# MuMuJun97/semantic_slam_mapping

Hardware: AMD Instinct MI355X
Metric: frames/sec semantic-mapping, 640x480 RGB-D (higher is better)
Workload: dtype u8; 1 GPU; configs[1]: synthetic 640x480 RGB-D + precomputed 12-class masks, 1k frames per GPU, ORB 1000 kp/frame, 5 ref frames, leaf 0.10 m; frames_per_gpu=1000, frames_all_gpus=1000, batch_frames=250, matcher_halo_frames=0, parallelism=single GPU

## Files before the change

### semantic_slam_mapping_amd/csrc/kernels_map.hip

```cpp
#include "ssm_internal.h"
#include <cstring>
#include <cmath>

#define MK_W 64
#define MK_H 16
__global__ void __launch_bounds__(256)
mask_kernel(const uint8_t* __restrict__ sem, int w, int h, int tiles_x, uint8_t* __restrict__ mask)
{
    __shared__ uint8_t m0[MK_H + 4][MK_W + 4];
    __shared__ uint8_t m1[MK_H + 4][MK_W];
    const int tx0 = (blockIdx.x % tiles_x) * MK_W, ty0 = (blockIdx.x / tiles_x) * MK_H;
    const uint8_t* s = sem + (size_t)blockIdx.y * w * h * 3;
    for (int i = threadIdx.x; i < (MK_H + 4) * (MK_W + 4); i += 256) {
        const int ly = i / (MK_W + 4), lx = i - ly * (MK_W + 4);
        const int gx = tx0 + lx - 2, gy = ty0 + ly - 2;
        uint8_t v = 0;
        if (gx >= 0 && gx < w && gy >= 0 && gy < h) {
            const uint8_t* p = s + ((size_t)gy * w + gx) * 3;
            const int b = p[0], g = p[1], r = p[2];
            v = ((b == 0 && g == 64 && r == 64) || (b == 192 && g == 128 && r == 0)) ? 255 : 0;
        }
        m0[ly][lx] = v;
    }
    __syncthreads();
// ... 311 lines not shown
    vox_insert_kernel<<<(int)blocks, 256, 0, s>>>(pts, n_dev, n_max, 1.0f / leaf, tab, cap_log2, counters);
    return hipGetLastError();
}
template <int CTRL, int ROW_MASK>
__device__ __forceinline__ int dpp_mov0(int v) { return __builtin_amdgcn_update_dpp(0, v, CTRL, ROW_MASK, 0xF, false); }
template <int CTRL, int ROW_MASK>
__device__ __forceinline__ long long dpp_mov0_ll(long long v)
{
    const int lo = dpp_mov0<CTRL, ROW_MASK>((int)(unsigned)(unsigned long long)v), hi = dpp_mov0<CTRL, ROW_MASK>((int)((unsigned long long)v >> 32));
    return (long long)(((unsigned long long)(unsigned)hi << 32) | (unsigned)lo);
}
struct RunAcc { long long sx, sy, sz; uint32_t r, g, b, n; };
__device__ __forceinline__ void run_scan(RunAcc& a, int lane, int start)
{
#define RS_STEP(CTRL, MASK, COND)                                                                                   \
    {   const long long tx = dpp_mov0_ll<CTRL, MASK>(a.sx), ty = dpp_mov0_ll<CTRL, MASK>(a.sy), tz = dpp_mov0_ll<CTRL, MASK>(a.sz); \
        const uint32_t t1 = (uint32_t)dpp_mov0<CTRL, MASK>((int)a.r), t2 = (uint32_t)dpp_mov0<CTRL, MASK>((int)a.g);             \
        const uint32_t t3 = (uint32_t)dpp_mov0<CTRL, MASK>((int)a.b), t4 = (uint32_t)dpp_mov0<CTRL, MASK>((int)a.n);             \
        if (COND) { a.sx += tx; a.sy += ty; a.sz += tz; a.r += t1; a.g += t2; a.b += t3; a.n += t4; } }
    const int li = lane & 15, row = lane >> 4;
    RS_STEP(0x111, 0xF, (li >= 1 && lane - 1 >= start))
    RS_STEP(0x112, 0xF, (li >= 2 && lane - 2 >= start))
    RS_STEP(0x114, 0xF, (li >= 4 && lane - 4 >= start))
    RS_STEP(0x118, 0xF, (li >= 8 && lane - 8 >= start))
    RS_STEP(0x142, 0xA, ((row & 1) && start < 16 * row))
    RS_STEP(0x143, 0xC, (row >= 2 && start < 32))
#undef RS_STEP
}
__device__ __forceinline__ long long f64_to_ll_rn(double v)
{
    const double M = 6755399441055744.0;
    return __double_as_longlong(v + M) - __double_as_longlong(M);
}
__device__ __forceinline__ uint32_t label_hash_entry(int k)
{
    switch (k) {
        case 10: return (0u << 24) | 128u | (128u << 8) | (128u << 16);   case 1:  return (1u << 24) | 0u | (0u << 8) | (128u << 16);
        case 2:  return (2u << 24) | 128u | (192u << 8) | (192u << 16);   case 9:  return (3u << 24) | 0u | (69u << 8) | (255u << 16);
        case 4:  return (4u << 24) | 128u | (64u << 8) | (128u << 16);    case 13: return (5u << 24) | 222u | (40u << 8) | (60u << 16);
        case 14: return (6u << 24) | 0u | (128u << 8) | (128u << 16);     case 11: return (7u << 24) | 128u | (128u << 8) | (192u << 16);
        case 3:  return (8u << 24) | 128u | (64u << 8) | (64u << 16);     case 12: return (9u << 24) | 128u | (0u << 8) | (64u << 16);
        case 7:  return (10u << 24) | 0u | (64u << 8) | (64u << 16);      case 15: return (11u << 24) | 192u | (128u << 8) | (0u << 16);
    }
    return 0xFF000001u;
}
#define MS_SLOTS 256
#ifndef MS_MINB
#define MS_MINB 4
#endif
#define MS_CH 3
struct LdsVox { long long key, sx, sy, sz; unsigned r, g, b, n; unsigned hist[6]; };
__device__ __forceinline__ uint32_t label_of_bgr24(uint32_t bgr)
{
    switch (bgr) {
        case 128u | (128u << 8) | (128u << 16): return 0;   case 0u | (0u << 8) | (128u << 16): return 1;
        case 128u | (192u << 8) | (192u << 16): return 2;   case 0u | (69u << 8) | (255u << 16): return 3;
        case 128u | (64u << 8) | (128u << 16): return 4;    case 222u | (40u << 8) | (60u << 16): return 5;
        case 0u | (128u << 8) | (128u << 16): return 6;     case 128u | (128u << 8) | (192u << 16): return 7;
        case 128u | (64u << 8) | (64u << 16): return 8;     case 128u | (0u << 8) | (64u << 16): return 9;
        case 0u | (64u << 8) | (64u << 16): return 10;      case 192u | (128u << 8) | (0u << 16): return 11;
    }
    return 255;
}
__device__ __forceinline__ void vox_direct(long long key, uint32_t lab, long long sx, long long sy, long long sz, unsigned r, unsigned g, unsigned b, unsigned n,
                ssm_voxel* tab, int cap_log2, int32_t* counters, uint32_t* occ)
{
// ... 98 lines not shown
            const int i = j < own0 ? j : j + (own1 - own0);
            const int rr = (int)__umulhi((uint32_t)i, mul_wpr), gy = ry0 + rr;
            uint32_t bits = 0;
            if (gy >= 0 && gy < h) {
                const uint4* p = reinterpret_cast<const uint4*>(sem + ((size_t)by * words + (size_t)((long long)ry0 * wpr + i)) * 48);
                const uint4 a = p[0], b = p[1], c = p[2];
                const uint32_t d[13] = {a.x, a.y, a.z, a.w, b.x, b.y, b.z, b.w, c.x, c.y, c.z, c.w, 0u};
#pragma unroll
                for (int k = 0; k < 16; k++) {
                    const int o = 3 * k;
                    const uint32_t bgr = ((o & 3) ? __builtin_amdgcn_alignbyte(d[(o >> 2) + 1], d[o >> 2], o & 3) : d[o >> 2]) & 0xFFFFFFu;
                    bits |= (uint32_t)(bgr == (0u | (64u << 8) | (64u << 16)) || bgr == (192u | (128u << 8) | (0u << 16))) << k;
                }
            }
            cbits[i] = (uint16_t)bits;
        }
    }
    for (int i = tid; i < MS_SLOTS; i += 256) {
        lt[i].key = SSM_VOX_EMPTY; lt[i].sx = 0; lt[i].sy = 0; lt[i].sz = 0; lt[i].r = lt[i].g = lt[i].b = lt[i].n = 0;
#pragma unroll
        for (int k = 0; k < 6; k++) lt[i].hist[k] = 0;
    }
    if (tid == 0) s_npts = 0;
    __syncthreads();
    if (!REDO && s_skip) return;
    uint32_t* occ = reinterpret_cast<uint32_t*>(tab + (1u << cap_log2));
    int kept = 0; bool out_of_range = false;
    double T[12];
    const bool hasT = pose != nullptr;
    if (hasT) { const double* P = pose + (size_t)by * 16;
#pragma unroll
        for (int j = 0; j < 4; j++) { T[3*j] = P[4*j]; T[3*j+1] = P[4*j+1]; T[3*j+2] = P[4*j+2]; } }
    const int dmax = maxd >= 65535.0 ? 65535 : (int)maxd;
#pragma unroll 1
    for (int ch = 0; ch < MS_CH; ch++) {
    const int wbase = (bx * MS_CH + ch) * 256 + wv * 64;
    const int wi = wbase + lane;
    uint32_t keepbits = 0;
    uint32_t lab4[2] = {labs[0][0], labs[0][1]};
#pragma unroll
    for (int c_ = 1; c_ < MS_CH; c_++) { lab4[0] = ch == c_ ? labs[c_][0] : lab4[0]; lab4[1] = ch == c_ ? labs[c_][1] : lab4[1]; }
    if (wi < words) {
        const size_t gw = (size_t)by * words + wi;
        const int gy = (int)__umulhi((uint32_t)wi, mul_wpr), xw = wi - gy * wpr;
        const uint4* pd = reinterpret_cast<const uint4*>(depth + gw * 16);
        const uint4 D0 = pd[0], D1 = pd[1];
        const uint16_t* cb = cbits + (gy - ry0 - 2) * wpr + xw;
        uint32_t vl = 0, vc = 0, vr = 0;
#pragma unroll
        for (int r5 = 0; r5 < 5; r5++) { vc |= cb[r5 * wpr]; if (xw > 0) vl |= cb[r5 * wpr - 1]; if (xw + 1 < wpr) vr |= cb[r5 * wpr + 1]; }
        const unsigned long long win = (unsigned long long)vl | ((unsigned long long)vc << 16) | ((unsigned long long)vr << 32);
        const uint32_t moving = (uint32_t)((win >> 14) | (win >> 15) | (win >> 16) | (win >> 17) | (win >> 18)) & 0xFFFFu;
        const uint32_t dd[8] = {D0.x, D0.y, D0.z, D0.w, D1.x, D1.y, D1.z, D1.w};
#pragma unroll
        for (int k = 0; k < 16; k++) {
            const int d = (dd[k >> 1] >> (16 * (k & 1))) & 0xFFFF;
            const uint32_t lab = (lab4[k >> 3] >> (4 * (k & 7))) & 15u;
            const bool gated = (0x805u >> lab) & 1u;
            keepbits |= (uint32_t)(d != 0 && d <= dmax && !gated) << k;
        }
        keepbits &= ~moving;
    }
    const uint32_t cnt = __popc(keepbits);
    uint32_t incl = cnt;
    incl += (uint32_t)__builtin_amdgcn_update_dpp(0, (int)incl, 0x111, 0xF, 0xF, false);
    incl += (uint32_t)__builtin_amdgcn_update_dpp(0, (int)incl, 0x112, 0xF, 0xF, false);
    incl += (uint32_t)__builtin_amdgcn_update_dpp(0, (int)incl, 0x114, 0xF, 0xF, false);
    incl += (uint32_t)__builtin_amdgcn_update_dpp(0, (int)incl, 0x118, 0xF, 0xF, false);
    incl += (uint32_t)__builtin_amdgcn_update_dpp(0, (int)incl, 0x142, 0xA, 0xF, false);
    incl += (uint32_t)__builtin_amdgcn_update_dpp(0, (int)incl, 0x143, 0xC, 0xF, false);
    const int V = __builtin_amdgcn_readlane((int)incl, 63);
    kept += (int)cnt;
    {
        int base = (int)(incl - cnt);
#pragma unroll
        for (int k = 0; k < 16; k++)
            if ((keepbits >> k) & 1u) vlist[wv][base++] = (uint16_t)((lane << 4) | k | (((lab4[k >> 3] >> (4 * (k & 7))) & 15u) << 10));
    }
    const int P = (V + 63) >> 6;
    long long k0 = -2, k1 = -2; uint32_t l0 = 255, l1 = 255; RunAcc a0, a1;
    a0.sx = a0.sy = a0.sz = 0; a0.r = a0.g = a0.b = a0.n = 0; a1 = a0;
    __builtin_amdgcn_wave_barrier();
    struct PixIn { uint32_t ent; int d; uint32_t c01, c2; };
    auto fetch = [&](int e, PixIn& q) {
        q.ent = vlist[wv][min(e, V - 1)];
        const int sl = (q.ent >> 4) & 63, k = q.ent & 15;
        const size_t gp = ((size_t)by * words + wbase + sl) * 16 + k;
        q.d = depth[gp];
        uint16_t c01; __builtin_memcpy(&c01, rgb + gp * 3, 2);
        q.c01 = c01; q.c2 = rgb[gp * 3 + 2];
    };
    auto pixel = [&](int e, const PixIn& q, long long& key, uint32_t& lab, RunAcc& p) {
        const uint32_t ent = q.ent;
        const int sl = (ent >> 4) & 63, k = ent & 15;
        lab = (ent >> 10) == 15u ? 255u : (ent >> 10);
        const int d = q.d;
        const uint32_t cbgr = q.c01 | (q.c2 << 16);
        const int wip = wbase + sl;
        const int gy = (int)__umulhi((uint32_t)wip, mul_wpr), gx = ((wip - gy * wpr) << 4) + k;
        const double yf = (double)gy - cam.cy;
        float x, y, z;
        if (FASTDIV) {
            z = (float)markstein_div((double)d, cam.scale, md.rscale);
            x = (float)markstein_div(((double)gx - cam.cx) * (double)z, cam.fx, md.rfx);
            y = (float)markstein_div(yf * (double)z, cam.fy, md.rfy);
        } else {
            z = (float)((double)d / cam.scale);
            x = (float)(((double)gx - cam.cx) * (double)z / cam.fx);
            y = (float)(yf * (double)z / cam.fy);
        }
        float ox = x, oy = y, oz = z;
        if (hasT) {
            const double X = x, Y = y, Z = z;
            ox = (float)(T[0] * X + T[3] * Y + T[6] * Z + T[9]);
            oy = (float)(T[1] * X + T[4] * Y + T[7] * Z + T[10]);
            oz = (float)(T[2] * X + T[5] * Y + T[8] * Z + T[11]);
        }
        const float fi = floorf(ox * inv_leaf), fj = floorf(oy * inv_leaf), fk = floorf(oz * inv_leaf);
        const long long vi = (long long)(int)fi + (1 << 20), vj = (long long)(int)fj + (1 << 20), vk = (long long)(int)fk + (1 << 20);
        key = (vk << 42) | (vj << 21) | vi;
        if (!(fabsf(fi) < 1048576.0f && fabsf(fj) < 1048576.0f && fabsf(fk) < 1048576.0f)) { key = -1; if (e < V) out_of_range = true; }
        p.sx = f64_to_ll_rn((double)ox * 16777216.0); p.sy = f64_to_ll_rn((double)oy * 16777216.0); p.sz = f64_to_ll_rn((double)oz * 16777216.0);
        p.b = cbgr & 255; p.g = (cbgr >> 8) & 255; p.r = cbgr >> 16; p.n = 1;
    };
    auto accumulate = [&](long long key, uint32_t lab, const RunAcc& p) {
        if (k1 == -2 && (k0 == -2 || (k0 == key && l0 == lab))) {
            k0 = key; l0 = lab; a0.sx += p.sx; a0.sy += p.sy; a0.sz += p.sz; a0.r += p.r; a0.g += p.g; a0.b += p.b; a0.n += 1;
        } else if (k1 == -2 || (k1 == key && l1 == lab)) {
            k1 = key; l1 = lab; a1.sx += p.sx; a1.sy += p.sy; a1.sz += p.sz; a1.r += p.r; a1.g += p.g; a1.b += p.b; a1.n += 1;
        } else {
            if (k1 >= 0) lds_vox_update(lt, k1, l1, a1, tab, cap_log2, counters, occ);
            k1 = key; l1 = lab; a1 = p;
        }
    };
    constexpr int MS2_UN = 2;
    PixIn cur[MS2_UN], nxt[MS2_UN];
    if (P > 0) {
#pragma unroll
        for (int u = 0; u < MS2_UN; u++) fetch(lane * P + u, nxt[u]);
    }
#pragma unroll 1
    for (int i = 0; i < P; i += MS2_UN) {
        long long kk[MS2_UN]; uint32_t ll[MS2_UN]; RunAcc pp[MS2_UN];
#pragma unroll
        for (int u = 0; u < MS2_UN; u++) { cur[u] = nxt[u]; fetch(lane * P + i + MS2_UN + u, nxt[u]); }
#pragma unroll
        for (int u = 0; u < MS2_UN; u++) pixel(lane * P + i + u, cur[u], kk[u], ll[u], pp[u]);
#pragma unroll
        for (int u = 0; u < MS2_UN; u++) if (i + u < P && lane * P + i + u < V) accumulate(kk[u], ll[u], pp[u]);
    }
    if (k0 >= 0) lds_vox_update(lt, k0, l0, a0, tab, cap_log2, counters, occ);
    if (k1 >= 0) lds_vox_update(lt, k1, l1, a1, tab, cap_log2, counters, occ);
    __builtin_amdgcn_wave_barrier();
    }
#pragma unroll
    for (int o = 32; o > 0; o >>= 1) kept += __shfl_xor(kept, o, 64);
    if (lane == 0 && kept) atomicAdd(&s_npts, kept);
    if (__ballot(out_of_range) && lane == 0) atomicOr(&counters[1], 2);
    __syncthreads();
    for (int i = tid; i < MS_SLOTS; i += 256) {
        if (lt[i].key == SSM_VOX_EMPTY) continue;
        ssm_voxel* v = vox_find_or_insert(tab, cap_log2, lt[i].key, counters, occ);
        if (__builtin_expect(!v, 0)) { vox_overflow_packed(counters, lt[i].key, lt[i].sx, lt[i].sy, lt[i].sz, lt[i].r, lt[i].g, lt[i].b, lt[i].n, lt[i].hist); continue; }
        vox_add(v, lt[i].sx, lt[i].sy, lt[i].sz, lt[i].r, lt[i].g, lt[i].b, lt[i].n);
#pragma unroll
        for (int c = 0; c < 12; c++) { const uint32_t k = (lt[i].hist[c >> 1] >> (16 * (c & 1))) & 0xFFFF; if (k) atomicAdd(&v->hist[c], k); }
    }
    if (tid == 0 && s_npts) atomicAdd(&npoints[by], s_npts);
}
bool k_map_div(const ssm_camera& cam, MapDiv& md)
{
    md.rscale = 1.0 / cam.scale; md.rfx = 1.0 / cam.fx; md.rfy = 1.0 / cam.fy;
    auto plain = [](double f) {
        uint64_t b; memcpy(&b, &f, 8);
        const uint64_t man = b & 0xFFFFFFFFFFFFFull; const int ex = (int)((b >> 52) & 0x7FF);
        return f > 0 && ex > 0 && ex < 0x7FF && man != 0xFFFFFFFFFFFFFull;
    };
    bool ok = plain(cam.scale) && plain(cam.fx) && plain(cam.fy);
    for (int d = 0; d < 65536 && ok; d++) {
        double q = (double)d * md.rscale; q = std::fma(std::fma(-q, cam.scale, (double)d), md.rscale, q); q = std::fma(std::fma(-q, cam.scale, (double)d), md.rscale, q);
        if (q != (double)d / cam.scale) ok = false;
    }
    return ok;
}
int k_map_fuse_blocks_per_frame(int w, int h) { const int words = (w >> 4) * h; return (words + 256 * MS_CH - 1) / (256 * MS_CH); }
int k_map_fuse_block_records(void) { return MS_CH * 4096; }
int k_map_fuse_resident_blocks(void) { return 256 * MS2_MINB; }
int k_map_fuse_skip_cap(void) { return MS2_SKIP_CAP; }
hipError_t k_map_fuse(const uint16_t* depth, const uint8_t* rgb, const uint8_t* sem, const double* pose, int n, int w, int h,
                      ssm_camera cam, const MapDiv& md, bool fast, double max_distance, float leaf,
                      ssm_voxel* tab, int cap_log2, int32_t* counters, int32_t* npoints, hipStream_t s, int32_t* skip, int hw, int tag, const int32_t* redo_ids, int nredo)
{
    const int wpr = w >> 4, words = wpr * h;
    if (!((long long)words * wpr < (1ll << 32) && wpr <= 256)) return hipErrorInvalidValue;
    if (nredo <= 0) { const hipError_t e = hipMemsetAsync(npoints, 0, sizeof(int32_t) * n, s); if (e != hipSuccess) return e; }
    const int gx = (words + 256 * MS_CH - 1) / (256 * MS_CH);
    const dim3 grid(gx, n);
    const uint32_t mul_wpr = (uint32_t)(((1ull << 32) + wpr - 1) / wpr);
    const double maxd = max_distance * cam.scale; const float il = 1.0f / leaf;
    if (nredo > 0) {
        int32_t* ids = const_cast<int32_t*>(redo_ids);
        if (fast) map_stream2_kernel<true, true><<<nredo, 256, 0, s>>>(depth, rgb, sem, pose, w, h, cam, md, maxd, il, tab, cap_log2, counters, npoints, mul_wpr, ids, 0, tag, gx);
        else map_stream2_kernel<false, true><<<nredo, 256, 0, s>>>(depth, rgb, sem, pose, w, h, cam, md, maxd, il, tab, cap_log2, counters, npoints, mul_wpr, ids, 0, tag, gx);
    } else {
        if (fast) map_stream2_kernel<true, false><<<grid, 256, 0, s>>>(depth, rgb, sem, pose, w, h, cam, md, maxd, il, tab, cap_log2, counters, npoints, mul_wpr, skip, hw, tag, gx);
        else map_stream2_kernel<false, false><<<grid, 256, 0, s>>>(depth, rgb, sem, pose, w, h, cam, md, maxd, il, tab, cap_log2, counters, npoints, mul_wpr, skip, hw, tag, gx);
    }
    return hipGetLastError();
}

__global__ void vox_merge_kernel(const ssm_voxel* __restrict__ src, int n, ssm_voxel* __restrict__ tab, int cap_log2, int32_t* __restrict__ counters)
{
    uint32_t* occ = reinterpret_cast<uint32_t*>(tab + (1u << cap_log2));
    const int i = blockIdx.x * blockDim.x + threadIdx.x;
    if (i >= n) return;
    const ssm_voxel sv = src[i];
    ssm_voxel* v = vox_find_or_insert(tab, cap_log2, sv.key, counters, occ);
    if (!v) { if (g_voxel* o = vox_overflow_slot(counters)) vox_store_record(o, sv); return; }
    vox_add(v, sv.sx, sv.sy, sv.sz, sv.sr, sv.sg, sv.sb, sv.n);
    for (int c = 0; c < 12; c++) if (sv.hist[c]) atomicAdd(&v->hist[c], sv.hist[c]);
// ... 135 lines not shown
```

### semantic_slam_mapping_amd/csrc/ssm_abi.hip

```cpp
#include "ssm_ctx.h"
#include <set>

static const int8_t k_default_pattern[1024] = {
#include "orb_pattern.inc"
};
thread_local std::string g_create_err;

static int fast_scored_cells(int a, int b, int n, int origin, int cell)
{
    const int s0 = a - 1 > SSM_EDGE ? a - 1 : SSM_EDGE, s1 = (b + 1 < n - SSM_EDGE ? b + 1 : n - SSM_EDGE) - 1;
    return (s1 - origin - 3) / cell - (s0 - origin - 3) / cell + 1;
}
static int build_geometry(const ssm_config& c, OrbGeom& g, std::string& err)
{
    memset(&g, 0, sizeof(g));
    if (c.orb_levels < 1 || c.orb_levels > SSM_MAX_LEVELS) { err = "orb_levels must be 1..12"; return SSM_E_INVAL; }
    if (c.orb_features < 1) { err = "orb_features must be >= 1"; return SSM_E_INVAL; }
    if (c.orb_iniThFAST < 1 || c.orb_minThFAST < 1 || c.orb_minThFAST > 254 || c.orb_iniThFAST > 254) { err = "FAST thresholds must be 1..254"; return SSM_E_INVAL; }
    if (c.width < 64 || c.height < 64 || c.width > 4000 || c.height > 4000) { err = "frame size must be 64..4000"; return SSM_E_INVAL; }
    if (!(c.orb_scale > 1.0f)) { err = "orb_scale must be > 1"; return SSM_E_INVAL; }
    g.nlevels = c.orb_levels; g.W = c.width; g.H = c.height; g.ini_th = c.orb_iniThFAST; g.min_th = c.orb_minThFAST;
    const double scaleFactor = (double)c.orb_scale;
    float sf[SSM_MAX_LEVELS], inv[SSM_MAX_LEVELS];
    sf[0] = 1.0f;
// ... 136 lines not shown
}

extern "C" void ssm_config_default(ssm_config* c)
{
    memset(c, 0, sizeof(*c));
    c->width = 640; c->height = 480;
    c->orb_features = 2000; c->orb_scale = 1.2f; c->orb_levels = 8; c->orb_iniThFAST = 20; c->orb_minThFAST = 7;
    c->knn_match_ratio = 0.8; c->tracker_ref_frames = 5;
    c->mapper_resolution = 0.1; c->mapper_max_distance = 40;
    c->camera.cx = 318.6; c->camera.cy = 255.3; c->camera.fx = 517.3; c->camera.fy = 516.5; c->camera.scale = 1000.0;
    c->max_batch = 16; c->voxel_capacity_log2 = 20; c->brief_pattern = nullptr;
    c->voxel_max_capacity_log2 = 28; c->sgbm_form = 0; c->sgbm_streams = 0; c->stereo_batch = 0;
}
extern "C" const char* ssm_version(void) { return "ssm_hip 0.1 (gfx950)"; }
extern "C" const char* ssm_last_error(const ssm_ctx* c) { return c ? c->err.c_str() : g_create_err.c_str(); }

static int orb_work_alloc(ssm_ctx* c, OrbWork& w)
{
    const OrbGeom& g = c->g; const int B = c->B;
    DALLOC(c, w.pyr, (size_t)B * g.pyr_bytes + 16); DALLOC(c, w.blur, (size_t)B * g.blur_bytes);
    DALLOC(c, w.ncand, k_fast_ncand_pad(B, g) + k_fast_cellmax_ints(B, g)); w.cellmax = w.ncand + k_fast_ncand_pad(B, g);
    DALLOC(c, w.cand, (size_t)B * g.cand_total); DALLOC(c, w.nodeof, (size_t)B * g.cand_total);
    DALLOC(c, w.sel, (size_t)B * g.sel_total); DALLOC(c, w.nsel, (size_t)B * g.nlevels);
    DALLOC(c, w.kpaux, (size_t)B * g.sel_total * 2);
    return SSM_OK;
}
static int ctx_init(ssm_ctx* c)
{
    const ssm_config& cfg = c->cfg; const OrbGeom& g = c->g; const int B = c->B, W = g.W, H = g.H;
    HIPCHK(c, c->main.stream.ensure());
    c->dev.id = c->device;
    { int v = 0; if (hipDeviceGetAttribute(&v, hipDeviceAttributeMultiprocessorCount, c->device) == hipSuccess && v > 0) c->dev.cus = v; }
    { int v = 0; if (hipDeviceGetAttribute(&v, hipDeviceAttributeMaxSharedMemoryPerBlock, c->device) == hipSuccess && v > 0) c->dev.max_lds = v; }
    c->map_div_exact = k_map_div(cfg.camera, c->map_div);
    DALLOC(c, c->d_pattern, 1024);
    HIPCHK(c, hipMemcpy(c->d_pattern, cfg.brief_pattern ? cfg.brief_pattern : k_default_pattern, 1024, hipMemcpyHostToDevice));
    {   float pf[1024]; const int8_t* src = cfg.brief_pattern ? cfg.brief_pattern : k_default_pattern;
        for (int i = 0; i < 1024; i++) pf[i] = (float)src[i];
        { const char* e = getenv("SSM_BLUR_VARIANT"); c->blur_mfma = !(e && atoi(e) == 0); }
        { std::vector<uint8_t> bt(blur_mfma_table_bytes(c->g)); blur_mfma_tables(c->g, bt.data());
          DALLOC(c, c->d_blur_tab, bt.size());
          HIPCHK(c, hipMemcpy(c->d_blur_tab, bt.data(), bt.size(), hipMemcpyHostToDevice)); }
        DALLOC(c, c->d_pattern_f, 1024);
        HIPCHK(c, hipMemcpy(c->d_pattern_f, pf, sizeof(pf), hipMemcpyHostToDevice)); }
    std::vector<int32_t> yall[SSM_MAX_LEVELS]; bool streaming[SSM_MAX_LEVELS] = {}, wide_ok[SSM_MAX_LEVELS] = {};
    for (int l = 1; l < g.nlevels; l++) {
        std::vector<int32_t> xo, yo; std::vector<int16_t> xa, ya;
        resize_tables(g.L[l-1].w, g.L[l].w, xo, xa); resize_tables(g.L[l-1].h, g.L[l].h, yo, ya);
        yall[l] = yo;
        std::vector<uint32_t> xg, xg8; bool fits = false, fits8 = false;
        pyramid_xgroups(xo, xa, ya, g.L[l].w, g.L[l].stride, g.L[l-1].stride, xg, xg8, fits, fits8);
        while (yo.size() & 3) { yo.push_back(yo.back()); ya.push_back(ya[ya.size() - 2]); ya.push_back(ya[ya.size() - 2]); }
        DALLOC(c, c->d_xofs[l], xo.size()); DALLOC(c, c->d_xa[l], xa.size()); DALLOC(c, c->d_yofs[l], yo.size()); DALLOC(c, c->d_ya[l], ya.size());
        HIPCHK(c, hipMemcpy(c->d_xofs[l], xo.data(), xo.size() * 4, hipMemcpyHostToDevice));
        HIPCHK(c, hipMemcpy(c->d_xa[l], xa.data(), xa.size() * 2, hipMemcpyHostToDevice));
        HIPCHK(c, hipMemcpy(c->d_yofs[l], yo.data(), yo.size() * 4, hipMemcpyHostToDevice));
        HIPCHK(c, hipMemcpy(c->d_ya[l], ya.data(), ya.size() * 2, hipMemcpyHostToDevice));
        if (fits) {
            DALLOC(c, c->d_xgrp[l], xg.size());
            HIPCHK(c, hipMemcpy(c->d_xgrp[l], xg.data(), xg.size() * 4, hipMemcpyHostToDevice));
            streaming[l] = true;
        }
        if (fits && fits8) {
            DALLOC(c, c->d_xgrp8[l], xg8.size());
            HIPCHK(c, hipMemcpy(c->d_xgrp8[l], xg8.data(), xg8.size() * 4, hipMemcpyHostToDevice));
            wide_ok[l] = true;
// ... 813 lines not shown
```

### semantic_slam_mapping_amd/csrc/ssm_internal.h

```cpp
#pragma once
#include <hip/hip_runtime.h>
#include <stdint.h>
#include <vector>
#include "../../include/ssm_hip.h"

#define SSM_MAX_LEVELS 12
#define SSM_EDGE 19
#define SSM_HALF_PATCH 15
#define SSM_PATCH 31
#define SSM_MAX_NODES 1024
#define SSM_VOX_EMPTY ((int64_t)-1)

struct LevelGeom {
    int w, h, stride;
    int img_off;
    int nCols, nRows, wCell, hCell;
    int cell_off;
    int tile_off, tiles_x;
    int ftile_off, ftiles_x;
    int ftw, fth;
    int nfeat;
    int cand_off, cand_cap;
    int sel_off, sel_cap;
    int minBX, minBY, maxBX, maxBY;
// ... 4 lines not shown
    int boff;
    int bt_off, bt_x, bt_units_off;
    uint32_t mulW, mulH;
};
__host__ __device__ inline int blur_off(int boff, int stride, int x, int y) { return boff + (((y >> 3) * (stride >> 4) + (x >> 4)) << 7) + ((y & 7) << 4) + (x & 15); }
#define FT_W 126
#define FT_H 32
#define FT_SW (FT_W + 2)
#define FT_SH (FT_H + 2)
#define FT_PW 144
#define FT_PH (FT_SH + 6)
#define FT_SST 132
#define FT_BW 32
#define FT_STAGE ((FT_PH * FT_PW) / 8)
#define FT_LDS_BYTES (4 * 8 + FT_PH * FT_PW + (FT_SH + 2) * FT_SST + 2 * FT_SW * FT_SH + 2 * (FT_SW + 2) + 2 * (FT_SH + 2) + 4 * 64 + 4 * 4 + 4 * 3)
__host__ __device__ inline void ftile_rect(const LevelGeom& L, int tx, int ty, int& x0, int& x1, int& y0, int& y1)
{
    x0 = SSM_EDGE + tx * L.ftw; x1 = x0 + L.ftw < L.w - SSM_EDGE ? x0 + L.ftw : L.w - SSM_EDGE;
    y0 = SSM_EDGE + ty * L.fth; y1 = y0 + L.fth < L.h - SSM_EDGE ? y0 + L.fth : L.h - SSM_EDGE;
}
struct OrbGeom {
    int nlevels, W, H;
    int pyr_bytes;
    int cells_total, cand_total, sel_total, tiles_total, ftiles_total;
    int blur_bytes;
    int bt_total, bt_units_total;
    int cap;
    int ini_th, min_th;
    int umax[SSM_HALF_PATCH + 1];
    LevelGeom L[SSM_MAX_LEVELS];
};
typedef uint2 cand_t;

struct DeviceInfo { int id = 0, cus = 256, max_lds = 160 * 1024; };
hipError_t allow_dynamic_lds(const void* fn, size_t bytes, int limit);

hipError_t k_gray(const uint8_t* img, int channels, int n, const OrbGeom& g, uint8_t* pyr, hipStream_t s);
hipError_t k_copy_gray_strided(const uint8_t* img, int stride, const OrbGeom& g, uint8_t* pyr, hipStream_t s);
hipError_t k_pyramid(int n, const OrbGeom& g, uint8_t* pyr, const int32_t* const* xofs, const int16_t* const* xa,
                     const int32_t* const* yofs, const int16_t* const* ya, const void* const* xgroups, hipStream_t s);
#define PB_MAX_LDS (80 * 1024)
struct PyrBandArgs {
    const void* xg[SSM_MAX_LEVELS]; const int32_t* yofs[SSM_MAX_LEVELS]; const int16_t* ya[SSM_MAX_LEVELS]; uint32_t mulq0, mulg[SSM_MAX_LEVELS]; int buf1;
    uint32_t wide;
};
__host__ __device__ inline int pyr_wide(const PyrBandArgs& t, int l) { return (int)(t.wide >> l) & 1; }
struct PyrBandPlan { int bands = 0; size_t lds = 0; void* d_tab = nullptr; PyrBandArgs args = {}; };
struct PyrItems { int groups, c0, nblk, items; };
__host__ __device__ inline PyrItems pyr_items(int stride, int wide, int comp_lo, int comp_hi)
{
    PyrItems it; it.groups = stride >> (wide ? 3 : 2); it.c0 = comp_lo & ~3; it.nblk = ((comp_hi - it.c0) >> 2) + 1;
    it.items = it.groups * it.nblk;
    return it;
}
__host__ __device__ inline int pyr_item_run(int i, uint32_t mulg) { return (int)(((uint64_t)(uint32_t)i * mulg) >> 32); }
#define PYR_SLACK 16
void pyramid_xgroups(const std::vector<int32_t>& xo, const std::vector<int16_t>& xa, const std::vector<int16_t>& ya, int dw, int dstride, int sstride,
                     std::vector<uint32_t>& xg4, std::vector<uint32_t>& xg8, bool& fits4, bool& fits8);
bool pyramid_band_choose(const OrbGeom& g, const std::vector<int32_t>* yofs, const bool* streaming, const bool* wide_ok, bool batch, std::vector<int32_t>& tab, PyrBandPlan& p);
bool pyramid_band_plan(const OrbGeom& g, const std::vector<int32_t>* yofs, const bool* streaming, const bool* wide_ok, int bands, std::vector<int32_t>& tab, PyrBandPlan& p);
hipError_t k_pyramid_bands(const uint8_t* img, int channels, int n, const OrbGeom& g, uint8_t* pyr, const PyrBandPlan& p,
                           const int32_t* const* yofs, const int16_t* const* ya, const void* const* xgroups, const void* const* xgroups8, hipStream_t s);
int pyramid_block_threads();
hipError_t k_blur(int n, const OrbGeom& g, const uint8_t* pyr, uint8_t* blur, hipStream_t s);
#define BLUR_ROWS 58
hipError_t k_blur_mfma(int n, const OrbGeom& g, const uint8_t* pyr, uint8_t* blur, const void* tab, hipStream_t s);
size_t blur_mfma_table_bytes(const OrbGeom& g);
// ... 5 lines not shown
                    uint32_t* sel, int32_t* nsel, int32_t* status, hipStream_t s);
hipError_t k_describe(int n, const OrbGeom& g, const uint8_t* pyr, const uint8_t* blur, const uint32_t* sel,
                      const int32_t* nsel, const float* pattern_f , const uint16_t* depth, ssm_camera cam, void* kpaux ,
                      ssm_keypoint* kps, uint8_t* desc, float* pos3d, int32_t* nkp, hipStream_t s);

struct MatchPair { int32_t qoff, nq, toff, nt, out_slot; };
hipError_t k_match_pairs(const uint8_t* desc, const MatchPair* pairs, int npairs, double ratio, int cap,
                         ssm_dmatch* out, int32_t* nout, int32_t* knn_idx, int32_t* knn_dist, hipStream_t s);
hipError_t k_match_seq(const uint8_t* desc, const int32_t* nkp, int f0, int n, int R, int hist, double ratio, int cap,
                       ssm_dmatch* out, int32_t* nout, int32_t* pend , hipStream_t s);

#define SSM_MATCH_DESC_BYTES 128
hipError_t k_match_expand(const uint8_t* desc, const int32_t* nkp, int row0, int nrows, int cap, int capT, uint8_t* eq, uint8_t* et, hipStream_t s);
hipError_t k_match_seq_mfma(const uint8_t* eq, const uint8_t* et, const int32_t* nkp, int f0, int n, int R, int hist, double ratio, int cap, int capT,
                            void* knn , ssm_dmatch* out, int32_t* nout, hipStream_t s);

hipError_t k_moving_mask(const uint8_t* sem, int n, int w, int h, uint8_t* mask, hipStream_t s);
hipError_t k_backproject(const uint16_t* depth, const uint8_t* rgb, const uint8_t* sem, const uint8_t* mask,
                         const double* pose, int n, int w, int h, ssm_camera cam, double max_distance,
                         int32_t* chunk_cnt, int64_t* chunk_off, int32_t* npoints, int64_t* total,
                         ssm_point* out, hipStream_t s);
int backproject_chunks(int w, int h);

hipError_t k_voxel_clear(ssm_voxel* tab, int cap_log2, int32_t* counters, hipStream_t s);
hipError_t k_voxel_insert(const ssm_point* pts, const int64_t* n_dev, int64_t n_max, float leaf, ssm_voxel* tab,
                          int cap_log2, int32_t* counters, hipStream_t s);
struct MapDiv { double rscale, rfx, rfy; };
bool k_map_div(const ssm_camera& cam, MapDiv& md);
hipError_t k_map_fuse(const uint16_t* depth, const uint8_t* rgb, const uint8_t* sem, const double* pose, int n, int w, int h,
                      ssm_camera cam, const MapDiv& md, bool exact, double max_distance, float leaf,
                      ssm_voxel* tab, int cap_log2, int32_t* counters, int32_t* npoints, hipStream_t s, int32_t* skip, int hw, int tag, const int32_t* redo_ids, int nredo);
int k_map_fuse_blocks_per_frame(int w, int h);
int k_map_fuse_block_records(void);
int k_map_fuse_resident_blocks(void);
int k_map_fuse_skip_cap(void);
hipError_t k_voxel_merge(const ssm_voxel* src, int n, ssm_voxel* tab, int cap_log2, int32_t* counters, hipStream_t s);
hipError_t k_voxel_rehash(const ssm_voxel* src, int src_cap_log2, ssm_voxel* tab, int cap_log2, int32_t* counters, hipStream_t s);
hipError_t k_voxel_compact(const ssm_voxel* tab, int cap_log2, ssm_voxel* out, int32_t* n_out, hipStream_t s);
hipError_t k_voxel_gather_points(const ssm_voxel* compact, const uint32_t* order, int n, ssm_point* out, hipStream_t s);
hipError_t k_voxel_gather_table(const ssm_voxel* compact, const uint32_t* order, int n, ssm_voxel* out, hipStream_t s);
hipError_t k_voxel_bounds(const ssm_point* pts, int n, float* minmax6, hipStream_t s);
hipError_t k_cloud_transform(const ssm_point* src, int n, const double* T, ssm_point* dst, hipStream_t s);
hipError_t voxel_sort_pairs(void* tmp, size_t* tmp_bytes, const ssm_voxel* compact, int n, uint64_t* keys_a, uint64_t* keys_b,
                            uint32_t* idx_a, uint32_t* idx_b, hipStream_t s);

hipError_t k_synth(uint64_t seed, int first, int n, int w, int h, uint8_t* bgr, uint16_t* depth, uint8_t* sem,
                   uint8_t* lab, double* pose, hipStream_t s);

hipError_t k_segnet_prep(const uint8_t* bgr, int n, int sw, int sh, int dw, int dh, const int32_t* xofs, const int16_t* xa,
                         const int32_t* yofs, const int16_t* ya, void* out_f16, hipStream_t s);
#define CONV_QUEUE_INTS 1024
hipError_t k_segnet_begin(int* tiles, hipStream_t s);
hipError_t k_segnet_conv(const void* in, const void* wt, const float* scale, const float* shift, void* out, int n, int H, int W,
                         int CinPad, int Cout, int relu, const DeviceInfo& dev, int* tiles, hipStream_t s, const void* wt_wino = nullptr);
size_t k_sgbm_workspace_bytes(int w, int h, const ssm_sgbm_params& p, int nb, int form_cfg);
bool sgbm_cost_geometry(int D, int SW, int* TX_out, size_t* lds_out);
struct SgFan;
hipError_t k_sgbm(const uint8_t* left, const uint8_t* right, int w, int h, int nb, const ssm_sgbm_params& p, void* workspace, size_t ws_bytes, int16_t* disp_out, int raw_only,
                  const DeviceInfo& dev, SgFan& fan, hipStream_t s, int* fail_flag = nullptr, int form_cfg = 0, int concurrent = 1);
hipError_t k_sgbm_post(const int16_t* src, int16_t* dst, int w, int h, int nb, int op, int newVal, int maxSpeckleSize, int maxDiff, int* parent, int* count, hipStream_t s);
hipError_t k_sgbm_depth(const int16_t* disp, int w, int h, int nb, double baseline, double cu, double cv, double f, double roix, double roiy, double roiz, double scale,
                        int* min_scratch , uint16_t* depth, hipStream_t s);
hipError_t k_vo_estimate(const ssm_pmatch* m, int n, const ssm_vo_params& P, const int32_t* samples, int iters,
                         double* tr_all, int32_t* count, double* tr_out, int32_t* inliers, int32_t* result, hipStream_t s);
hipError_t k_vo_estimate_batch(const ssm_pmatch* m_all, int stride, const int32_t* n_all, int nb, const ssm_vo_params& P, const uint32_t* rand_stream, int iters,
                               int32_t* consumed, int32_t* rand_off, double* tr_all, int32_t* count, double* tr_out, int32_t* inliers, int32_t* result, hipStream_t s);
hipError_t k_segnet_conv_argmax(const void* in, const void* wt, const float* scale, const float* shift, uint8_t* labels, int n, int H, int W,
// ... 37 lines not shown
```

### semantic_slam_mapping_amd/csrc/ssm_map.hip

```cpp
#include "ssm_ctx.h"
#include <algorithm>

int table_alloc(ssm_ctx* c, hipStream_t s, VoxTable& t, int cap_log2, const VoxTable* lists)
{
    if (!lists) lists = &t;
    t.cap_log2 = cap_log2;
    { const int r = t.tab.alloc_bytes(c, t.bytes()); if (r) return r; }
    const size_t slots = (size_t)1 << cap_log2;
    t.occ = reinterpret_cast<uint32_t*>(t.tab + slots); t.counters = reinterpret_cast<int32_t*>(t.occ + slots);
    HIPCHK(c, k_voxel_clear(t.tab, -cap_log2, t.counters, s));
    struct { int32_t cap, pad; ssm_voxel* buf; } tail = { lists->ovf ? lists->ovf_cap : 0, 0, lists->ovf };
    static_assert(sizeof(tail) == 16, "counter block tail");
    int32_t head[3] = {0, 0, 0};
    HIPCHK(c, hipMemcpyAsync(t.counters, head, 12, hipMemcpyHostToDevice, s));
    HIPCHK(c, hipMemcpyAsync(t.counters + 3, &tail.cap, 4, hipMemcpyHostToDevice, s));
    HIPCHK(c, hipMemcpyAsync(t.counters + 4, &tail.buf, 8, hipMemcpyHostToDevice, s));
    HIPCHK(c, hipStreamSynchronize(s));
    return SSM_OK;
}
static int map_drain_other_streams(ssm_ctx* c, hipStream_t s)
{
    for (hipStream_t st : c->map_launch_streams) if (st && st != s) HIPCHK(c, hipStreamSynchronize(st));
    return SSM_OK;
}
static int64_t map_stream_list_records()
{
    const char* e = getenv("SSM_MAP_TEST_SMALL_LIST"); const bool small = e && atoi(e) != 0;
    return small ? (int64_t)VOX_OVF_RECORDS : (int64_t)VOX_OVF_RECORDS + (int64_t)k_map_fuse_resident_blocks() * k_map_fuse_block_records();
}
static int map_ensure_stream_list(ssm_ctx* c, hipStream_t s)
{
    VoxTable& t = c->map;
    if (t.skip && t.ovf_cap >= map_stream_list_records()) return SSM_OK;
    int r = map_settle(c, s, 0); if (r) return r;
    if (!t.skip) { DALLOC(c, t.skip, (size_t)k_map_fuse_skip_cap()); DALLOC(c, c->d_redo, (size_t)k_map_fuse_skip_cap()); }
    if (t.ovf_cap < map_stream_list_records()) {
        DevBuf<ssm_voxel> big;
        DALLOC(c, big, (size_t)map_stream_list_records());
        t.ovf = std::move(big); t.ovf_cap = (int)map_stream_list_records();
        struct { int32_t cap, pad; ssm_voxel* buf; } tail = { t.ovf_cap, 0, t.ovf };
        HIPCHK(c, hipMemcpyAsync(t.counters + 3, &tail.cap, 4, hipMemcpyHostToDevice, s));
        HIPCHK(c, hipMemcpyAsync(t.counters + 4, &tail.buf, 8, hipMemcpyHostToDevice, s));
        HIPCHK(c, hipStreamSynchronize(s));
    }
    return SSM_OK;
}
int map_fuse_launch(ssm_ctx* c, hipStream_t s, const MapLaunch& L)
{
    VoxTable& t = c->map;
    int r = map_ensure_stream_list(c, s); if (r) return r;
    const int gx = k_map_fuse_blocks_per_frame(L.w, L.h);
    if ((int64_t)gx * L.n > k_map_fuse_skip_cap() / 4) FAIL(c, SSM_E_INVAL, "map stage: more than " + std::to_string(k_map_fuse_skip_cap() / 4) + " blocks in one launch (frames per launch x frame size)");
    const int64_t resident = std::min<int64_t>(k_map_fuse_resident_blocks(), (int64_t)gx * L.n);
    const int64_t hw = (int64_t)t.ovf_cap - resident * k_map_fuse_block_records();
    const int tag = (int)(c->map_ring_next++ & 7u);
    c->map_ring[tag] = L; c->map_ring[tag].valid = true;
    c->map_unexamined = true;
    if (std::find(c->map_launch_streams.begin(), c->map_launch_streams.end(), s) == c->map_launch_streams.end()) c->map_launch_streams.push_back(s);
    HIPCHK(c, k_map_fuse(L.depth, L.rgb, L.sem, L.pose, L.n, L.w, L.h, c->cfg.camera, c->map_div, c->map_div_exact, c->cfg.mapper_max_distance, (float)c->cfg.mapper_resolution,
                         t.tab, t.cap_log2, t.counters, L.npoints, s, t.skip, (int)hw, tag, nullptr, 0));
    return SSM_OK;
}
int map_settle(ssm_ctx* c, hipStream_t s, int64_t reserve, int32_t* counters_out)
{
    VoxTable& t = c->map;
    int lo = 0;
    for (int round = 0; round < 4096; round++) {
        int32_t cnt[8];
        HIPCHK(c, hipMemcpyAsync(cnt, t.counters, 32, hipMemcpyDeviceToHost, s));
        HIPCHK(c, hipStreamSynchronize(s));
        if (c->map_unexamined || cnt[6] > 0) {
            { const int r = map_drain_other_streams(c, s); if (r) return r; }
            HIPCHK(c, hipMemcpyAsync(cnt, t.counters, 32, hipMemcpyDeviceToHost, s)); HIPCHK(c, hipStreamSynchronize(s));
            c->map_unexamined = false;
        }
        if (cnt[6] > 0) {
            const int ns = cnt[6] < k_map_fuse_skip_cap() ? cnt[6] : k_map_fuse_skip_cap();
            const size_t at = c->map_skipped.size(); c->map_skipped.resize(at + (size_t)ns);
            const int32_t z = 0;
            HIPCHK(c, hipMemcpyAsync(c->map_skipped.data() + at, t.skip, (size_t)ns * 4, hipMemcpyDeviceToHost, s));
            HIPCHK(c, hipMemcpyAsync(t.counters + 6, &z, 4, hipMemcpyHostToDevice, s)); HIPCHK(c, hipStreamSynchronize(s));
            cnt[6] = 0;
        }
        const int64_t n = cnt[0], hi = cnt[2] < t.ovf_cap ? cnt[2] : t.ovf_cap, m = hi - lo;
        const int64_t slots = (int64_t)1 << t.cap_log2;
        const bool grow = 4 * (n + m + reserve) > slots && t.cap_log2 < c->vox_max_log2;
// ... 519 lines not shown
```

Baseline: 185,000 frames/s.

## Accumulate voxel runs via prefix sums with biased fixed-point and query real occupancy

Replaces the per-pixel two-slot run accumulator with one running prefix sum per lane. Positions are converted to fixed point with a single fma plus magic bias, and B/R colour channels are packed into one 32-bit word. Run totals are recovered by subtracting a saved base and the accumulated bias, which removes branchy per-field adds in the inner loop. Separately, the resident-block estimate used to size the overflow list now comes from the occupancy API instead of a constant, which changes the reserved headroom.

```diff
diff --git a/semantic_slam_mapping_amd/csrc/kernels_map.hip b/semantic_slam_mapping_amd/csrc/kernels_map.hip
--- a/semantic_slam_mapping_amd/csrc/kernels_map.hip
+++ b/semantic_slam_mapping_amd/csrc/kernels_map.hip
@@ -367,6 +367,30 @@
     const double M = 6755399441055744.0;
     return __double_as_longlong(v + M) - __double_as_longlong(M);
 }
+struct FixedK { double scale, magic; };
+__device__ __forceinline__ unsigned long long raw_fixed(float v, const FixedK& K)
+{
+    return (unsigned long long)__double_as_longlong(fma((double)v, K.scale, K.magic));
+}
+__device__ __forceinline__ FixedK fixed_consts()
+{
+    FixedK K = { 16777216.0, 6755399441055744.0 };
+    asm volatile("" : "+s"(K.scale), "+v"(K.magic));
+    return K;
+}
+struct RunSum { unsigned long long sx, sy, sz; uint32_t br, g; };
+__device__ __forceinline__ RunSum run_diff(const RunSum& s, const RunSum& b)
+{
+    RunSum d; d.sx = s.sx - b.sx; d.sy = s.sy - b.sy; d.sz = s.sz - b.sz; d.br = s.br - b.br; d.g = s.g - b.g;
+    return d;
+}
+__device__ __forceinline__ RunAcc run_total(const RunSum& d, uint32_t n)
+{
+    const unsigned long long bias = (unsigned long long)n * (unsigned long long)__double_as_longlong(6755399441055744.0);
+    RunAcc f; f.sx = (long long)(d.sx - bias); f.sy = (long long)(d.sy - bias); f.sz = (long long)(d.sz - bias);
+    f.b = d.br & 0xFFFFu; f.r = d.br >> 16; f.g = d.g; f.n = n;
+    return f;
+}
 __device__ __forceinline__ uint32_t label_hash_entry(int k)
 {
     switch (k) {
@@ -531,6 +555,7 @@
 #pragma unroll
         for (int j = 0; j < 4; j++) { T[3*j] = P[4*j]; T[3*j+1] = P[4*j+1]; T[3*j+2] = P[4*j+2]; } }
     const int dmax = maxd >= 65535.0 ? 65535 : (int)maxd;
+    const FixedK fixk = fixed_consts();
 #pragma unroll 1
     for (int ch = 0; ch < MS_CH; ch++) {
     const int wbase = (bx * MS_CH + ch) * 256 + wv * 64;
@@ -577,24 +602,24 @@
             if ((keepbits >> k) & 1u) vlist[wv][base++] = (uint16_t)((lane << 4) | k | (((lab4[k >> 3] >> (4 * (k & 7))) & 15u) << 10));
     }
     const int P = (V + 63) >> 6;
-    long long k0 = -2, k1 = -2; uint32_t l0 = 255, l1 = 255; RunAcc a0, a1;
-    a0.sx = a0.sy = a0.sz = 0; a0.r = a0.g = a0.b = a0.n = 0; a1 = a0;
+    RunSum S, B;
+    S.sx = S.sy = S.sz = 0; S.br = S.g = 0; B = S;
+    long long k0 = -2, kc = -2; uint32_t l0 = 255, lc = 255; int nb = 0;
     __builtin_amdgcn_wave_barrier();
-    struct PixIn { uint32_t ent; int d; uint32_t c01, c2; };
+    struct PixIn { uint32_t ent; int d; uint32_t bgr; };
     auto fetch = [&](int e, PixIn& q) {
         q.ent = vlist[wv][min(e, V - 1)];
         const int sl = (q.ent >> 4) & 63, k = q.ent & 15;
         const size_t gp = ((size_t)by * words + wbase + sl) * 16 + k;
         q.d = depth[gp];
         uint16_t c01; __builtin_memcpy(&c01, rgb + gp * 3, 2);
-        q.c01 = c01; q.c2 = rgb[gp * 3 + 2];
+        q.bgr = (uint32_t)c01 | ((uint32_t)rgb[gp * 3 + 2] << 16);
     };
-    auto pixel = [&](int e, const PixIn& q, long long& key, uint32_t& lab, RunAcc& p) {
+    auto pixel = [&](int e, const PixIn& q, long long& key, uint32_t& lab, RunSum& p) {
         const uint32_t ent = q.ent;
         const int sl = (ent >> 4) & 63, k = ent & 15;
         lab = (ent >> 10) == 15u ? 255u : (ent >> 10);
         const int d = q.d;
-        const uint32_t cbgr = q.c01 | (q.c2 << 16);
         const int wip = wbase + sl;
         const int gy = (int)__umulhi((uint32_t)wip, mul_wpr), gx = ((wip - gy * wpr) << 4) + k;
         const double yf = (double)gy - cam.cy;
@@ -619,18 +644,24 @@
         const long long vi = (long long)(int)fi + (1 << 20), vj = (long long)(int)fj + (1 << 20), vk = (long long)(int)fk + (1 << 20);
         key = (vk << 42) | (vj << 21) | vi;
         if (!(fabsf(fi) < 1048576.0f && fabsf(fj) < 1048576.0f && fabsf(fk) < 1048576.0f)) { key = -1; if (e < V) out_of_range = true; }
-        p.sx = f64_to_ll_rn((double)ox * 16777216.0); p.sy = f64_to_ll_rn((double)oy * 16777216.0); p.sz = f64_to_ll_rn((double)oz * 16777216.0);
-        p.b = cbgr & 255; p.g = (cbgr >> 8) & 255; p.r = cbgr >> 16; p.n = 1;
+        p.sx = raw_fixed(ox, fixk); p.sy = raw_fixed(oy, fixk); p.sz = raw_fixed(oz, fixk);
+        p.br = q.bgr & 0x00FF00FFu;
+        p.g = (q.bgr >> 8) & 255u;
     };
-    auto accumulate = [&](long long key, uint32_t lab, const RunAcc& p) {
-        if (k1 == -2 && (k0 == -2 || (k0 == key && l0 == lab))) {
-            k0 = key; l0 = lab; a0.sx += p.sx; a0.sy += p.sy; a0.sz += p.sz; a0.r += p.r; a0.g += p.g; a0.b += p.b; a0.n += 1;
-        } else if (k1 == -2 || (k1 == key && l1 == lab)) {
-            k1 = key; l1 = lab; a1.sx += p.sx; a1.sy += p.sy; a1.sz += p.sz; a1.r += p.r; a1.g += p.g; a1.b += p.b; a1.n += 1;
-        } else {
-            if (k1 >= 0) lds_vox_update(lt, k1, l1, a1, tab, cap_log2, counters, occ);
-            k1 = key; l1 = lab; a1 = p;
-        }
+    auto accumulate = [&](int j, long long key, uint32_t lab, const RunSum& p) {
+        if (key != kc || lab != lc) {
+            if (kc != -2) {
+                if (k0 == -2) { k0 = kc; l0 = lc; }
+                else {
+                    if (k0 >= 0) lds_vox_update(lt, k0, l0, run_total(B, (uint32_t)nb), tab, cap_log2, counters, occ);
+                    if (kc >= 0) lds_vox_update(lt, kc, lc, run_total(run_diff(S, B), (uint32_t)(j - nb)), tab, cap_log2, counters, occ);
+                    k0 = -3;
+                }
+                B = S; nb = j;
+            }
+            kc = key; lc = lab;
+        }
+        S.sx += p.sx; S.sy += p.sy; S.sz += p.sz; S.br += p.br; S.g += p.g;
     };
     constexpr int MS2_UN = 2;
     PixIn cur[MS2_UN], nxt[MS2_UN];
@@ -640,16 +671,16 @@
     }
 #pragma unroll 1
     for (int i = 0; i < P; i += MS2_UN) {
-        long long kk[MS2_UN]; uint32_t ll[MS2_UN]; RunAcc pp[MS2_UN];
+        long long kk[MS2_UN]; uint32_t ll[MS2_UN]; RunSum pp[MS2_UN];
 #pragma unroll
         for (int u = 0; u < MS2_UN; u++) { cur[u] = nxt[u]; fetch(lane * P + i + MS2_UN + u, nxt[u]); }
 #pragma unroll
         for (int u = 0; u < MS2_UN; u++) pixel(lane * P + i + u, cur[u], kk[u], ll[u], pp[u]);
 #pragma unroll
-        for (int u = 0; u < MS2_UN; u++) if (i + u < P && lane * P + i + u < V) accumulate(kk[u], ll[u], pp[u]);
-    }
-    if (k0 >= 0) lds_vox_update(lt, k0, l0, a0, tab, cap_log2, counters, occ);
-    if (k1 >= 0) lds_vox_update(lt, k1, l1, a1, tab, cap_log2, counters, occ);
+        for (int u = 0; u < MS2_UN; u++) if (i + u < P && lane * P + i + u < V) accumulate(i + u, kk[u], ll[u], pp[u]);
+    }
+    if (k0 >= 0) lds_vox_update(lt, k0, l0, run_total(B, (uint32_t)nb), tab, cap_log2, counters, occ);
+    if (kc >= 0) lds_vox_update(lt, kc, lc, run_total(run_diff(S, B), (uint32_t)(min(max(V - lane * P, 0), P) - nb)), tab, cap_log2, counters, occ);
     __builtin_amdgcn_wave_barrier();
     }
 #pragma unroll
@@ -684,7 +715,17 @@
 }
 int k_map_fuse_blocks_per_frame(int w, int h) { const int words = (w >> 4) * h; return (words + 256 * MS_CH - 1) / (256 * MS_CH); }
 int k_map_fuse_block_records(void) { return MS_CH * 4096; }
-int k_map_fuse_resident_blocks(void) { return 256 * MS2_MINB; }
+int k_map_fuse_resident_blocks(int cus)
+{
+    int per_cu = 0;
+    const void* kern[2] = { reinterpret_cast<const void*>(&map_stream2_kernel<true, false>), reinterpret_cast<const void*>(&map_stream2_kernel<false, false>) };
+    for (const void* k : kern) {
+        int nb = 0;
+        if (hipOccupancyMaxActiveBlocksPerMultiprocessor(&nb, k, 256, 0) != hipSuccess || nb <= 0) { (void)hipGetLastError(); nb = 8; }
+        per_cu = nb > per_cu ? nb : per_cu;
+    }
+    return cus * per_cu;
+}
 int k_map_fuse_skip_cap(void) { return MS2_SKIP_CAP; }
 hipError_t k_map_fuse(const uint16_t* depth, const uint8_t* rgb, const uint8_t* sem, const double* pose, int n, int w, int h,
                       ssm_camera cam, const MapDiv& md, bool fast, double max_distance, float leaf,
diff --git a/semantic_slam_mapping_amd/csrc/ssm_abi.hip b/semantic_slam_mapping_amd/csrc/ssm_abi.hip
--- a/semantic_slam_mapping_amd/csrc/ssm_abi.hip
+++ b/semantic_slam_mapping_amd/csrc/ssm_abi.hip
@@ -192,6 +192,7 @@
     c->dev.id = c->device;
     { int v = 0; if (hipDeviceGetAttribute(&v, hipDeviceAttributeMultiprocessorCount, c->device) == hipSuccess && v > 0) c->dev.cus = v; }
     { int v = 0; if (hipDeviceGetAttribute(&v, hipDeviceAttributeMaxSharedMemoryPerBlock, c->device) == hipSuccess && v > 0) c->dev.max_lds = v; }
+    c->dev.map_resident = k_map_fuse_resident_blocks(c->dev.cus);
     c->map_div_exact = k_map_div(cfg.camera, c->map_div);
     DALLOC(c, c->d_pattern, 1024);
     HIPCHK(c, hipMemcpy(c->d_pattern, cfg.brief_pattern ? cfg.brief_pattern : k_default_pattern, 1024, hipMemcpyHostToDevice));
diff --git a/semantic_slam_mapping_amd/csrc/ssm_internal.h b/semantic_slam_mapping_amd/csrc/ssm_internal.h
--- a/semantic_slam_mapping_amd/csrc/ssm_internal.h
+++ b/semantic_slam_mapping_amd/csrc/ssm_internal.h
@@ -60,7 +60,7 @@
 };
 typedef uint2 cand_t;
 
-struct DeviceInfo { int id = 0, cus = 256, max_lds = 160 * 1024; };
+struct DeviceInfo { int id = 0, cus = 256, max_lds = 160 * 1024, map_resident = 256 * 8; };
 hipError_t allow_dynamic_lds(const void* fn, size_t bytes, int limit);
 
 hipError_t k_gray(const uint8_t* img, int channels, int n, const OrbGeom& g, uint8_t* pyr, hipStream_t s);
@@ -132,7 +132,7 @@
                       ssm_voxel* tab, int cap_log2, int32_t* counters, int32_t* npoints, hipStream_t s, int32_t* skip, int hw, int tag, const int32_t* redo_ids, int nredo);
 int k_map_fuse_blocks_per_frame(int w, int h);
 int k_map_fuse_block_records(void);
-int k_map_fuse_resident_blocks(void);
+int k_map_fuse_resident_blocks(int cus);
 int k_map_fuse_skip_cap(void);
 hipError_t k_voxel_merge(const ssm_voxel* src, int n, ssm_voxel* tab, int cap_log2, int32_t* counters, hipStream_t s);
 hipError_t k_voxel_rehash(const ssm_voxel* src, int src_cap_log2, ssm_voxel* tab, int cap_log2, int32_t* counters, hipStream_t s);
diff --git a/semantic_slam_mapping_amd/csrc/ssm_map.hip b/semantic_slam_mapping_amd/csrc/ssm_map.hip
--- a/semantic_slam_mapping_amd/csrc/ssm_map.hip
+++ b/semantic_slam_mapping_amd/csrc/ssm_map.hip
@@ -23,21 +23,21 @@
     for (hipStream_t st : c->map_launch_streams) if (st && st != s) HIPCHK(c, hipStreamSynchronize(st));
     return SSM_OK;
 }
-static int64_t map_stream_list_records()
+static int64_t map_stream_list_records(const ssm_ctx* c)
 {
     const char* e = getenv("SSM_MAP_TEST_SMALL_LIST"); const bool small = e && atoi(e) != 0;
-    return small ? (int64_t)VOX_OVF_RECORDS : (int64_t)VOX_OVF_RECORDS + (int64_t)k_map_fuse_resident_blocks() * k_map_fuse_block_records();
+    return small ? (int64_t)VOX_OVF_RECORDS : (int64_t)VOX_OVF_RECORDS + (int64_t)c->dev.map_resident * k_map_fuse_block_records();
 }
 static int map_ensure_stream_list(ssm_ctx* c, hipStream_t s)
 {
     VoxTable& t = c->map;
-    if (t.skip && t.ovf_cap >= map_stream_list_records()) return SSM_OK;
+    if (t.skip && t.ovf_cap >= map_stream_list_records(c)) return SSM_OK;
     int r = map_settle(c, s, 0); if (r) return r;
     if (!t.skip) { DALLOC(c, t.skip, (size_t)k_map_fuse_skip_cap()); DALLOC(c, c->d_redo, (size_t)k_map_fuse_skip_cap()); }
-    if (t.ovf_cap < map_stream_list_records()) {
+    if (t.ovf_cap < map_stream_list_records(c)) {
         DevBuf<ssm_voxel> big;
-        DALLOC(c, big, (size_t)map_stream_list_records());
-        t.ovf = std::move(big); t.ovf_cap = (int)map_stream_list_records();
+        DALLOC(c, big, (size_t)map_stream_list_records(c));
+        t.ovf = std::move(big); t.ovf_cap = (int)map_stream_list_records(c);
         struct { int32_t cap, pad; ssm_voxel* buf; } tail = { t.ovf_cap, 0, t.ovf };
         HIPCHK(c, hipMemcpyAsync(t.counters + 3, &tail.cap, 4, hipMemcpyHostToDevice, s));
         HIPCHK(c, hipMemcpyAsync(t.counters + 4, &tail.buf, 8, hipMemcpyHostToDevice, s));
@@ -51,7 +51,7 @@
     int r = map_ensure_stream_list(c, s); if (r) return r;
     const int gx = k_map_fuse_blocks_per_frame(L.w, L.h);
     if ((int64_t)gx * L.n > k_map_fuse_skip_cap() / 4) FAIL(c, SSM_E_INVAL, "map stage: more than " + std::to_string(k_map_fuse_skip_cap() / 4) + " blocks in one launch (frames per launch x frame size)");
-    const int64_t resident = std::min<int64_t>(k_map_fuse_resident_blocks(), (int64_t)gx * L.n);
+    const int64_t resident = std::min<int64_t>(c->dev.map_resident, (int64_t)gx * L.n);
     const int64_t hw = (int64_t)t.ovf_cap - resident * k_map_fuse_block_records();
     const int tag = (int)(c->map_ring_next++ & 7u);
     c->map_ring[tag] = L; c->map_ring[tag].valid = true;
```

Result: slower. 183,100 frames/s (-1.0%).
